# algbio/founderblockgraphs

Measured on AMD Instinct MI355X. Metric: MSA columns segmented/sec, higher is better.
Workload: dtype u32

## Files before the change

founderblockgraphs_amd/csrc/ctx.hip:

```cpp
#include "fbg_internal.h"
#include <chrono>
#include <stdarg.h>
#include <stdio.h>
#include <ctype.h>
#include <string.h>
#include <algorithm>
#include <atomic>
#include <thread>
#include <vector>

static std::string g_global_err;

int fbg_fail(fbg_ctx *ctx, int code, const char *fmt, ...)
{
    char buf[1024];
    va_list ap;
    va_start(ap, fmt);
    vsnprintf(buf, sizeof(buf), fmt, ap);
    va_end(ap);
    if (ctx) ctx->err = buf; else g_global_err = buf;
    return code;
}

int fbg_reserve(fbg_ctx *ctx, DevBuf &b, size_t bytes, std::vector<DevBuf *> *owner, bool accounted)
// ... 177 lines not shown
    {"span_slow_split", &FbgOptions::span_slow_split},
    {"poison", &FbgOptions::poison},
    {"dpw_matrix", &FbgOptions::dpw_matrix},
    {"dp_chain1", &FbgOptions::dp_chain1},
    {"msd_ext", &FbgOptions::msd_ext},
    {"rows_wave", &FbgOptions::rows_wave},
    {"pairs_in_scan", &FbgOptions::pairs_in_scan},
    {"runs_wave_min", &FbgOptions::runs_wave_min},
    {"wave_list_cap", &FbgOptions::wave_list_cap},
    {"cand_local_sort", &FbgOptions::cand_local_sort},
    {"cand_lds_cap", &FbgOptions::cand_lds_cap},
    {"cand_sort_check", &FbgOptions::cand_sort_check},
    {"tie_gallop", &FbgOptions::tie_gallop},
    {"cand_counts_fused", &FbgOptions::cand_counts_fused},
    {"tie_sample_loop", &FbgOptions::tie_sample_loop},
};

struct InfoKey { const char *name; int64_t (*get)(const fbg_ctx &); };
static const InfoKey g_info_keys[] = {
    {"grs_threshold", [](const fbg_ctx &c) -> int64_t { return c.grs_t; }},
    {"grs_redone", [](const fbg_ctx &c) -> int64_t { return (int64_t)c.grs_redone; }},
    {"dp_kind", [](const fbg_ctx &c) -> int64_t { return c.dp_kind; }},
    {"msd_decline", [](const fbg_ctx &c) -> int64_t { return c.diag.msd_decline; }},
    {"pass1_ahead", [](const fbg_ctx &c) -> int64_t { return c.diag.pass1_ahead; }},
    {"ext_pairs", [](const fbg_ctx &c) -> int64_t { return c.diag.ext_pairs; }},
    {"text_pairs", [](const fbg_ctx &c) -> int64_t { return c.diag.text_pairs; }},
    {"cand_inversions", [](const fbg_ctx &c) -> int64_t { return c.diag.cand_inversions; }},
    {"cand_local_sorted", [](const fbg_ctx &c) -> int64_t { return c.diag.cand_local_sorted; }},
    {"wave_runs", [](const fbg_ctx &c) -> int64_t { return c.diag.wave_runs; }},
    {"rank_lean_used", [](const fbg_ctx &c) -> int64_t { return c.diag.rank_lean_used; }},
    {"rank_lean_launched", [](const fbg_ctx &c) -> int64_t { return c.diag.rank_lean_launched; }},
    {"pairs_rb", [](const fbg_ctx &c) -> int64_t { return c.diag.pairs_rb; }},
    {"key_b", [](const fbg_ctx &c) -> int64_t { return c.key_b; }},
    {"key_K", [](const fbg_ctx &c) -> int64_t { return c.key_K; }},
    {"key_packed", [](const fbg_ctx &c) -> int64_t { return c.key_packed; }},
    {"key_compact", [](const fbg_ctx &c) -> int64_t { return c.key_compact; }},
    {"alloc_calls", [](const fbg_ctx &c) -> int64_t { return (int64_t)c.alloc_calls; }},
    {"alloc_us", [](const fbg_ctx &c) -> int64_t { return (int64_t)c.alloc_us; }},
    {"span_decline", [](const fbg_ctx &c) -> int64_t { return c.diag.sp_decline; }},
    {"span_key_flags_used", [](const fbg_ctx &c) -> int64_t { return c.ix.index_valid && c.ix.spanned() && c.ix.sp_key_flags_sorted; }},
    {"span_scan_used", [](const fbg_ctx &c) -> int64_t { return c.ix.index_valid && c.ix.spanned(); }},
// ... 118 lines not shown
        (void)hipStreamSynchronize(ctx->up_stream);
        for (auto &e : ctx->up_ev) if (e) (void)hipEventDestroy(e);
        (void)hipStreamDestroy(ctx->up_stream);
    }
    for (auto &t : ctx->timers) {
        if (t.start) (void)hipEventDestroy(t.start);
        if (t.stop) (void)hipEventDestroy(t.stop);
    }
    if (ctx->stager.base) {
        for (int i = 0; i < ctx->stager.nslots; i++) (void)hipEventDestroy(ctx->stager.ev[i]);
        delete[] ctx->stager.ev;
        (void)hipStreamDestroy(ctx->stager.stream);
        (void)hipHostFree(ctx->stager.base);
    }
    if (ctx->pin_pair) (void)hipHostFree(ctx->pin_pair);
    if (ctx->aux_fork) (void)hipEventDestroy(ctx->aux_fork);
    if (ctx->aux_join) (void)hipEventDestroy(ctx->aux_join);
    if (ctx->aux) (void)hipStreamDestroy(ctx->aux);
    if (ctx->own_stream) (void)hipStreamDestroy(ctx->stream);
    delete ctx;
}

const char *fbg_last_error(const fbg_ctx *ctx) { return ctx ? ctx->err.c_str() : g_global_err.c_str(); }

int fbg_set_stream(fbg_ctx *ctx, void *hip_stream)
{
    if (!ctx) return FBG_ERR_INVALID;
    FBG_HIP_TRY(ctx, hipStreamSynchronize(ctx->stream));
    if (ctx->own_stream) { (void)hipStreamDestroy(ctx->stream); ctx->own_stream = false; }
    if (hip_stream) {
// ... 376 lines not shown
```

founderblockgraphs_amd/csrc/fbg_internal.h:

```cpp
#pragma once
#include <cstring>
#include <cstdlib>
#include <hip/hip_runtime.h>
#include <stdint.h>
#include <string>
#include <vector>
#include "../../include/fbg_hip.h"

#define FBG_WAVE 64

struct DevBuf {
    void *p = nullptr;
    size_t cap = 0;
    bool listed = false;
    template <class T> T *as() const { return reinterpret_cast<T *>(p); }
};

struct Stager {
    void *base = nullptr;
    size_t slot_bytes = 0;
    int nslots = 0;
    hipEvent_t *ev = nullptr;
    hipStream_t stream = nullptr;
};

struct StageTimer {
    hipEvent_t start = nullptr, stop = nullptr;
    bool recorded = false;
    int launches = 0;
};

struct FbgOptions {
    int64_t no_ranked = 0, no_packed = 0, force_wide = 0, full_keys = 0, no_msd_sort = 0, msd_min = -1, bp_min = -1,
            record_scatter = 0, lcp_text = 0, no_aux_stream = 0, rank_no_threshold = 0, dp_literal = 0, dp_wave = 0,
            dp_safe_window = 0, dp_tile = 0, pure_scan = 0, gapped_rank = 0, part_tricks_off = 0, msd_sample_bins = 0, msd_min_force = 0, msd_probe = 0, msd_xcd = -1, rank_no_lean = 0, no_stream_upload = 0,
            span_scan = 0, span_key_flags = 0, span_slow_split = 0, poison = 0, dpw_matrix = 0, dp_chain1 = 0, msd_ext = 1, rows_wave = 0,
            pairs_in_scan = 1, runs_wave_min = 16, wave_list_cap = 0,
            cand_local_sort = 1, cand_lds_cap = 0, cand_sort_check = 0,
            tie_gallop = 1, cand_counts_fused = 1, tie_sample_loop = 1;
};

enum class IndexKind { none, record, ranked, gapped, span };

struct IndexState {
    bool index_valid = false;
    IndexKind kind = IndexKind::none;
    bool ranked() const { return kind == IndexKind::ranked; }
    bool granked() const { return kind == IndexKind::gapped || kind == IndexKind::span; }
    bool spanned() const { return kind == IndexKind::span; }
    uint32_t *sa_ptr = nullptr;
    uint64_t *rk_keys = nullptr;
    int rk_b = 0, rk_key_bits = 0, rk_K = 0;
    int rk_layout = 0, rk_pb = 0;
    bool grs_flagged = false;
// ... 2 lines not shown
    bool lcp_from_keys = false;
    bool grs_ties_done = false;
    uint32_t n_exc = 0;
    bool part_active = false;
    bool gpart = false;
    int part = 0, nparts = 1;
    uint64_t part_count = 0;
    uint64_t part_T = 0;
    uint32_t part_gmin = 0;
};

struct BuildDiag {
    int64_t msd_decline = -1;
    int pass1_ahead = 0;
    int64_t ext_pairs = -1, text_pairs = -1;
    int64_t wave_runs = -1;
    int64_t cand_inversions = -1;
    int cand_local_sorted = -1;
    int rank_lean_launched = 0;
    int rank_lean_used = 0;
    int pairs_rb = -1;
    int sp_decline = 0;
};

struct SortExtras {
    const uint64_t *ebits = nullptr;
    const uint32_t *payload = nullptr;
    bool key_flags = false;
};

struct MsdPlan;
struct fbg_ctx {
    int device = 0;
    FbgOptions opt;
    std::string err;
    hipStream_t stream = nullptr;
    bool own_stream = false;
    hipStream_t aux = nullptr;
    hipEvent_t aux_fork = nullptr, aux_join = nullptr;
    bool aux_pending = false;
    uint32_t *pin_pair = nullptr;
    Stager stager;
    StageTimer timers[FBG_STAGE_COUNT];

    const uint8_t *d_msa = nullptr;
    DevBuf msa_own;
    uint64_t m = 0, n = 0;
    int reversed = 0;
    bool gapfree = true;
    bool have_ignore = false;
    uint8_t ignore_tab[256] = {0};
    uint64_t N = 0;
    uint64_t byte_hist[256] = {0};
    bool allow_wide = false;
    uint32_t mp = 0;
    DevBuf text;
// ... 173 lines not shown
```

founderblockgraphs_amd/csrc/host/host_selftest.cpp:

```cpp
#include <cstdio>
#include <cstdlib>
#include <string>
#include <vector>
#include "fasta.hpp"
#include "xgfa.hpp"
#include "../tie_extent.h"

static int tie_extent_selftest()
{
    const uint32_t cap = 8192;
    std::vector<uint32_t> sizes;
    for (uint32_t s = 1; s <= 70; s++) sizes.push_back(s);
    for (uint32_t s = 8191; s <= 8194; s++) sizes.push_back(s);
    unsigned long long cases = 0;
    for (const uint32_t s : sizes)
        for (int where = 0; where < 3; where++) {
            const uint64_t before = where == 0 ? 0 : 37, after = where == 2 ? 0 : 29;
            std::vector<uint64_t> keys;
            for (uint64_t i = 0; i < before; i++) keys.push_back(10 + i / 3);
            const uint64_t key = 1000;
            for (uint32_t i = 0; i < s; i++) keys.push_back(key);
            for (uint64_t i = 0; i < after; i++) keys.push_back(2000 + i / 2);
            const uint64_t k0 = before;
            uint64_t reads = 0;
// ... 10 lines not shown
                reads = 0;
                const uint32_t got = fbg_tie_extent(k0, hi, cap, key, key_at);
                const uint64_t most = FBG_TIE_PROBE + 2 * 14;
                if (got != want || reads > most) {
                    std::printf("tie_extent differs: size %u position %d hi %llu: got %u, want %u, %llu reads\n", s, where,
                                (unsigned long long)hi, got, want, (unsigned long long)reads);
                    return 1;
                }
                cases++;
            }
        }
    std::printf("tie_extent ok %llu\n", cases);
    return 0;
}

int main(int argc, char **argv)
{
    if (argc == 2 && std::string(argv[1]) == "tie-extent") return tie_extent_selftest();
    if (argc < 6) {
        std::fprintf(stderr, "usage: %s FASTA GAP_LIMIT ELASTIC PATHS OUT.gfa [BOUNDARY ...]\n", argv[0]);
        return 2;
    }
    Msa msa;
    if (!read_msa(argv[1], std::atol(argv[2]), std::atoi(argv[3]) != 0, std::atoi(argv[4]) != 0, msa)) {
        std::fprintf(stderr, "cannot read %s\n", argv[1]);
        return 3;
    }
    std::printf("%llu %llu\n", (unsigned long long)msa.m, (unsigned long long)msa.n);
    if (argc == 6 || msa.m == 0) return 0;
    std::vector<uint64_t> boundaries;
    int first_boundary = 6;
    BlockGraph g;
// ... 28 lines not shown
```

founderblockgraphs_amd/csrc/suffix_sort.hip:

```cpp
#include "fbg_internal.h"
#include "text_cmp.h"
#include <rocprim/rocprim.hpp>
#include <utility>
#include <cmath>

#define SS_THREADS 256

using fbg_sort_config = rocprim::radix_sort_config<
    rocprim::default_config, rocprim::default_config,
    rocprim::radix_sort_onesweep_config<rocprim::kernel_config<512, 32>, rocprim::kernel_config<1024, 8>, 9,
                                        rocprim::block_radix_rank_algorithm::match>>;

#define PK_ITEMS 8
#define FBG_SEP 0x80
struct PackArgs {
    const uint8_t *T;
    uint64_t N;
    const uint8_t *code;
    int b, K, pb;
    uint64_t *keys;
    uint32_t *vals;
    uint64_t lo, hi, cap;
    int nohi;
    unsigned long long *counter;
// ... 108 lines not shown
    a.ebits = x.ebits; a.payload = x.payload;
    a.key_flags = x.key_flags ? ctx->sp_flagT.as<uint8_t>() : nullptr;
    const dim3 grid(fbg_blocks(a.N, SS_THREADS * PK_ITEMS)), block(SS_THREADS);
    hipStream_t st = ctx->stream;
#define FBG_PACK(C, L, F) hipLaunchKernelGGL((k_pack<C, L, F>), grid, block, 0, st, a)
    if (g.compact) {
        if (g.packed) { if (filter) FBG_PACK(true, FBG_SLOTS_PACKED, true); else FBG_PACK(true, FBG_SLOTS_PACKED, false); }
        else if (g.wide) { if (filter) FBG_PACK(true, FBG_SLOTS_WIDE, true); else FBG_PACK(true, FBG_SLOTS_WIDE, false); }
        else { if (filter) FBG_PACK(true, FBG_SLOTS_PAIRS, true); else FBG_PACK(true, FBG_SLOTS_PAIRS, false); }
    } else {
        if (filter) FBG_PACK(false, FBG_SLOTS_PAIRS, true); else FBG_PACK(false, FBG_SLOTS_PAIRS, false);
    }
#undef FBG_PACK
}

__global__ void k_sample_keys(const uint8_t *__restrict__ T, uint64_t N, const uint8_t *__restrict__ code, int b, int K,
                              int compact, uint64_t stride, uint64_t S, uint64_t *__restrict__ out)
{
    __shared__ uint8_t cd[256];
    if (threadIdx.x < 256) cd[threadIdx.x] = code[threadIdx.x];
    __syncthreads();
    const uint64_t i = (uint64_t)blockIdx.x * blockDim.x + threadIdx.x;
    if (i >= S) return;
    const uint64_t p = i * stride;
    uint64_t key = 0;
    bool dead = false;
    for (int k0 = 0; k0 < K; k0 += 8) {
        const uint64_t x = p + k0 < N ? fbg_load8(T, p + k0) : 0ull;
        for (int k = k0; k < K && k < k0 + 8; k++) {
            const uint32_t c = p + k < N ? cd[(x >> (8 * (k - k0))) & 255u] : (compact ? FBG_SEP : 0);
            dead = dead || (compact && (c & FBG_SEP));
            key = (key << b) | (dead ? 0u : c);
        }
    }
    out[i] = key;
}

__global__ void k_count_equal_neighbours(const uint64_t *__restrict__ keys, uint64_t S, unsigned long long *__restrict__ out)
{
    const uint64_t i = (uint64_t)blockIdx.x * blockDim.x + threadIdx.x;
    const bool eq = i + 1 < S && keys[i] == keys[i + 1];
    __shared__ uint32_t blk;
    if (threadIdx.x == 0) blk = 0;
    __syncthreads();
    const unsigned long long m = __ballot(eq);
    if ((threadIdx.x & 63) == 0 && m) atomicAdd(&blk, (uint32_t)__popcll(m));
    __syncthreads();
    if (threadIdx.x == 0 && blk) atomicAdd(out, (unsigned long long)blk);
}

// ... 508 lines not shown
        const unsigned hi = (unsigned)(g.pb + g.key_bits);
        if (hi == 64 && count < (1u << 23)) lo = 0;
        return with_tmp(ctx, [&](void *tmp, size_t &bytes) {
            return rocprim::radix_sort_keys<fbg_sort_config>(tmp, bytes, ka, kb, (size_t)count, lo, hi, st);
        });
    }
    uint32_t *va = ctx->valsA.as<uint32_t>(), *vb = ctx->valsB.as<uint32_t>() + out_offset;
    unsigned lo = g.wide ? (unsigned)g.pb : key_flags ? 2u : 0u;
    const unsigned hi = lo + (unsigned)g.key_bits;
    if (hi == 64 && count < (1u << 23)) lo = 0;
    return with_tmp(ctx, [&](void *tmp, size_t &bytes) {
        return rocprim::radix_sort_pairs<fbg_sort_config>(tmp, bytes, ka, kb, va, vb, (size_t)count, lo, hi, st);
    });
}

static int sample_says_similar(fbg_ctx *ctx, const KeyGeom &g, bool *similar, int *launches)
{
    const uint64_t N = ctx->N;
    hipStream_t st = ctx->stream;
    *similar = false;
    if (N < (1u << 22)) return FBG_OK;
    const uint64_t S = 1u << 20, stride = N / S;
    FBG_TRY(fbg_reserve(ctx, ctx->dp_g, S * 8));
    FBG_TRY(fbg_reserve(ctx, ctx->dp_h, S * 8));
    uint64_t *smp = ctx->dp_g.as<uint64_t>(), *srt = ctx->dp_h.as<uint64_t>();
    unsigned long long *d_count = ctx->scalars.as<unsigned long long>() + 8;
    FBG_HIP_TRY(ctx, hipMemsetAsync(d_count, 0, 8, st));
    hipLaunchKernelGGL(k_sample_keys, dim3(fbg_blocks(S, 256)), dim3(256), 0, st, ctx->text.as<uint8_t>(), N, g.d_code, g.b, g.K,
                       g.compact ? 1 : 0, stride, S, smp);
    FBG_TRY(with_tmp(ctx, [&](void *tmp, size_t &bytes) {
        return rocprim::radix_sort_keys(tmp, bytes, smp, srt, (size_t)S, 0u, (unsigned)g.key_bits, st);
    }));
    hipLaunchKernelGGL(k_count_equal_neighbours, dim3(fbg_blocks(S, 256)), dim3(256), 0, st, srt, S, d_count);
    unsigned long long twins = 0;
    FBG_HIP_TRY(ctx, hipMemcpyAsync(&twins, d_count, 8, hipMemcpyDeviceToHost, st));
    FBG_HIP_TRY(ctx, hipStreamSynchronize(st));
    *launches += 3;
    const double est = (double)twins * (double)N / ((double)S * (double)S);
    *similar = est > 0.5;
    return FBG_OK;
}

int fbg_suffix_sort(fbg_ctx *ctx)
{
    const uint64_t N = ctx->N;
    hipStream_t st = ctx->stream;
    FBG_TRY(fbg_stage_begin(ctx, FBG_STAGE_SUFFIX_SORT));
    int launches = 0;
    const uint8_t *T = ctx->text.as<uint8_t>();
    KeyGeom g;
    SortExtras x;

    if (ctx->gapfree && !ctx->have_ignore && !ctx->opt.no_ranked) {
        if (!fbg_msd_pre_geom(ctx, &g)) FBG_TRY(fbg_key_setup(ctx, true, &g, &launches));
    }
    if (ctx->gapfree && !ctx->have_ignore && !ctx->opt.no_ranked && g.compact) {
        bool similar = false;
        FBG_TRY(sample_says_similar(ctx, g, &similar, &launches));
        uint64_t *sorted = nullptr;
        int msd_ok = 0;
        FBG_TRY(fbg_msd_sort(ctx, g, &sorted, &msd_ok, &launches));
        if (!msd_ok) {
            FBG_TRY(fbg_reserve(ctx, ctx->keysA, N * 8));
            FBG_TRY(fbg_reserve(ctx, ctx->keysB, N * 8));
            if (!g.packed) {
                FBG_TRY(fbg_reserve(ctx, ctx->valsA, N * 4));
                FBG_TRY(fbg_reserve(ctx, ctx->valsB, N * 4));
            }
            PackArgs pa;
            pa.T = T; pa.N = N; pa.code = g.d_code; pa.b = g.b; pa.K = g.K; pa.pb = g.pb;
            pa.keys = ctx->keysA.as<uint64_t>(); pa.vals = ctx->valsA.as<uint32_t>();
            pa.lo = pa.hi = pa.cap = 0; pa.nohi = 1; pa.counter = nullptr;
            launch_pack(ctx, g, false, pa, x);
            launches++;
            FBG_TRY(sort_slots(ctx, g, false, N, 0));
            sorted = ctx->keysB.as<uint64_t>();
        }
        uint32_t *svals = g.packed ? nullptr : ctx->valsB.as<uint32_t>();
        int done = 0;
        if (!similar && ctx->opt.pure_scan != 1) FBG_TRY(fbg_rank_scan_try(ctx, sorted, svals, g, &done));
        if (!done && ctx->opt.pure_scan != -1) FBG_TRY(fbg_pure_scan_try(ctx, sorted, svals, g, &done));
        if (done) {
            FBG_HIP_TRY(ctx, hipGetLastError());
            return fbg_stage_end(ctx, FBG_STAGE_SUFFIX_SORT, launches);
        }
    }

    FBG_TRY(fbg_key_setup(ctx, false, &g, &launches));
    int b = g.b, K = g.K, key_bits = g.key_bits;
    FBG_TRY(fbg_reserve(ctx, ctx->keysA, N * 8));
    FBG_TRY(fbg_reserve(ctx, ctx->keysB, N * 8));
    FBG_TRY(fbg_reserve(ctx, ctx->valsA, N * 4));
    FBG_TRY(fbg_reserve(ctx, ctx->valsB, N * 4));
// ... 282 lines not shown
```

founderblockgraphs_amd/csrc/text_build.hip:

```cpp
#include "fbg_internal.h"

#define TB_THREADS 256
#define TB_ITEMS 8
#define TB_CHUNK (TB_THREADS * TB_ITEMS)

__device__ __forceinline__ uint32_t wave_incl_scan(uint32_t v)
{
    const int lane = threadIdx.x & 63;
#pragma unroll
    for (int d = 1; d < 64; d <<= 1) {
        uint32_t o = __shfl_up(v, d, 64);
        if (lane >= d) v += o;
    }
    return v;
}

__device__ __forceinline__ uint32_t block_excl_scan(uint32_t v, uint32_t *total, uint32_t *lds4)
{
    const int lane = threadIdx.x & 63, w = threadIdx.x >> 6;
    uint32_t inc = wave_incl_scan(v);
    if (lane == 63) lds4[w] = inc;
    __syncthreads();
    uint32_t base = 0, tot = 0;
#pragma unroll
// ... 141 lines not shown
    }
    if (lane == 0) { red[0][threadIdx.x >> 6] = nongap; red[1][threadIdx.x >> 6] = ign; }
    __syncthreads();
    if (sh[threadIdx.x]) atomicAdd(&hist[threadIdx.x], (unsigned long long)sh[threadIdx.x]);
    if (T_copy && threadIdx.x == 1 && x_hi == n) T_copy[i * (n + 1) + n] = '#';
    if (threadIdx.x == 0) {
        uint32_t a = 0, b = 0;
        for (int k = 0; k < TB_THREADS / 64; k++) { a += red[0][k]; b += red[1][k]; }
        atomicAdd(&tot[i], a);
        segcnt[i * gridDim.x + blockIdx.x] = a;
        atomicAdd(&scalars[0], (unsigned long long)((x_hi > x_lo ? x_hi - x_lo : 0) - a));
        if (b) atomicAdd(&scalars[1], (unsigned long long)b);
    }
}

__global__ void k_row_offsets(const uint32_t *__restrict__ tot, uint64_t m, uint32_t *__restrict__ pos,
                              unsigned long long *__restrict__ scalars)
{
    if (blockIdx.x != 0 || threadIdx.x >= 64) return;
    const uint64_t per = (m + 63) / 64, lo = min(m, (uint64_t)threadIdx.x * per), hi = min(m, lo + per);
    unsigned long long mine = 0;
    for (uint64_t i = lo; i < hi; i++) mine += (unsigned long long)tot[i] + 1;
    unsigned long long inc = mine;
    for (int d = 1; d < 64; d <<= 1) { const unsigned long long o = __shfl_up(inc, d, 64); if ((int)threadIdx.x >= d) inc += o; }
    unsigned long long s = inc - mine;
    for (uint64_t i = lo; i < hi; i++) { pos[i] = (uint32_t)s; s += (unsigned long long)tot[i] + 1; }
    if (threadIdx.x == 63) scalars[2] = inc + 1;
}

__global__ void k_seg_offsets(const uint32_t *__restrict__ segcnt, uint64_t m, uint32_t nseg, uint32_t *__restrict__ segoff)
// ... 162 lines not shown
#pragma unroll
        for (int k = 0; k < TB_ITEMS; k++)
            if (x0 + k < x_hi) igrow[i * n + x0 + k] = min(loc[k], right);
        __syncthreads();
        carry = chunk_min;
    }
}

int fbg_build_text(fbg_ctx *ctx, const uint8_t *ignore, uint64_t ignore_len)
{
    const uint64_t m = ctx->m, n = ctx->n;
    hipStream_t st = ctx->stream;
    FBG_TRY(fbg_stage_begin(ctx, FBG_STAGE_TEXT));
    int launches = 0;
    FBG_TRY(fbg_reserve(ctx, ctx->pos, m * 4));
    FBG_TRY(fbg_reserve(ctx, ctx->tot, m * 4));
    FBG_TRY(fbg_reserve(ctx, ctx->scalars, 256 * sizeof(unsigned long long)));
    FBG_TRY(fbg_reserve(ctx, ctx->small, 8192));
    FBG_HIP_TRY(ctx, hipMemsetAsync(ctx->scalars.p, 0, 64 * sizeof(unsigned long long), st));

    ctx->have_ignore = ignore_len > 0;
    ctx->cells_built = false;
    memset(ctx->ignore_tab, 0, sizeof(ctx->ignore_tab));
    if (ctx->have_ignore) {
        for (uint64_t k = 0; k < ignore_len; k++) ctx->ignore_tab[ignore[k]] = 1;
        FBG_HIP_TRY(ctx, hipMemcpyAsync(ctx->small.as<uint8_t>(), ctx->ignore_tab, 256, hipMemcpyHostToDevice, st));
    }
    unsigned long long *sc = ctx->scalars.as<unsigned long long>();
    unsigned long long *d_hist = reinterpret_cast<unsigned long long *>(ctx->small.as<uint8_t>() + 4096);
    FBG_HIP_TRY(ctx, hipMemsetAsync(d_hist, 0, 2048, st));
    FBG_HIP_TRY(ctx, hipMemsetAsync(ctx->tot.p, 0, m * 4, st));
    const unsigned nseg = (unsigned)((n + RC_SEG - 1) / RC_SEG);
    FBG_TRY(fbg_reserve(ctx, ctx->segtab, (size_t)m * nseg * 4 * 3));
    uint32_t *segcnt = ctx->segtab.as<uint32_t>(), *segoff = segcnt + (size_t)m * nseg;
    const bool fused = !ctx->reversed && n % 8 == 0 && ((uintptr_t)ctx->d_msa & 7) == 0 && m * (n + 1) + 1 < (1ull << 40);
    if (fused) FBG_TRY(fbg_reserve(ctx, ctx->text, m * (n + 1) + 1 + 64));
    const uint8_t *up = ctx->up_host;
    ctx->up_host = nullptr;
    ctx->pre_pass1 = false;
    if (up && fused && m >= 16) {
        constexpr int CHUNKS = 8;
        if (!ctx->up_stream) {
            FBG_HIP_TRY(ctx, hipStreamCreateWithFlags(&ctx->up_stream, hipStreamNonBlocking));
            for (auto &e : ctx->up_ev) FBG_HIP_TRY(ctx, hipEventCreateWithFlags(&e, hipEventDisableTiming));
        }
        uint8_t *d_msa = ctx->msa_own.as<uint8_t>();
        FBG_HIP_TRY(ctx, hipEventRecord(ctx->up_ev[CHUNKS], st));
        FBG_HIP_TRY(ctx, hipStreamWaitEvent(ctx->up_stream, ctx->up_ev[CHUNKS], 0));
        uint64_t r0s[CHUNKS + 1];
        for (int c = 0; c <= CHUNKS; c++) r0s[c] = m * c / CHUNKS;
        for (int c = 0; c < CHUNKS; c++) {
            FBG_HIP_TRY(ctx, hipMemcpyAsync(d_msa + r0s[c] * n, up + r0s[c] * n, (r0s[c + 1] - r0s[c]) * n, hipMemcpyHostToDevice, ctx->up_stream));
            FBG_HIP_TRY(ctx, hipEventRecord(ctx->up_ev[c], ctx->up_stream));
        }
        bool pre = false;
        for (int c = 0; c < CHUNKS; c++) {
            FBG_HIP_TRY(ctx, hipStreamWaitEvent(st, ctx->up_ev[c], 0));
            hipLaunchKernelGGL(k_row_count, dim3(nseg, (unsigned)(r0s[c + 1] - r0s[c])), dim3(TB_THREADS), 0, st, ctx->d_msa,
                               n, (const uint8_t *)nullptr, ctx->tot.as<uint32_t>(), sc, d_hist, segcnt, ctx->text.as<uint8_t>(), (uint32_t)r0s[c]);
            if (c == 0) {
                unsigned long long h0[1];
                FBG_HIP_TRY(ctx, hipMemcpyAsync(h0, sc, sizeof(h0), hipMemcpyDeviceToHost, st));
                FBG_HIP_TRY(ctx, hipMemcpyAsync(ctx->byte_hist, d_hist, 256 * sizeof(uint64_t), hipMemcpyDeviceToHost, st));
                FBG_HIP_TRY(ctx, hipStreamSynchronize(st));
                if (h0[0] == 0) {
                    for (int b = 0; b < 256; b++) ctx->byte_hist[b] = ctx->byte_hist[b] * m / r0s[1];
                    ctx->byte_hist['-'] = 0; ctx->byte_hist['#'] += m; ctx->byte_hist[0] += 1;
                    ctx->N = m * (n + 1) + 1;
                    ctx->gapfree = true;
                    FBG_HIP_TRY(ctx, hipMemsetAsync(ctx->text.as<uint8_t>() + ctx->N - 1, 0, 65, st));
                    int ok = 0;
                    FBG_TRY(fbg_msd_pre_begin(ctx, &ok));
                    pre = ok != 0;
                }
            }
            if (pre) FBG_TRY(fbg_msd_pre_pass1(ctx, c + 1 < CHUNKS ? r0s[c + 1] * (n + 1) : ctx->N));
        }
        ctx->pre_pass1 = pre;
        launches += CHUNKS - 1;
    } else {
        if (up) FBG_TRY(fbg_upload(ctx, ctx->msa_own.p, up, m * n));
        hipLaunchKernelGGL(k_row_count, dim3(nseg, (unsigned)m), dim3(TB_THREADS), 0, st, ctx->d_msa,
                           n, (const uint8_t *)nullptr, ctx->tot.as<uint32_t>(), sc, d_hist, segcnt, fused ? ctx->text.as<uint8_t>() : (uint8_t *)nullptr);
    }
    hipLaunchKernelGGL(k_row_offsets, dim3(1), dim3(64), 0, st, ctx->tot.as<uint32_t>(), m,
                       ctx->pos.as<uint32_t>(), sc);
    launches += 2;
    unsigned long long h[3];
    FBG_HIP_TRY(ctx, hipMemcpyAsync(h, sc, sizeof(h), hipMemcpyDeviceToHost, st));
    FBG_HIP_TRY(ctx, hipMemcpyAsync(ctx->byte_hist, d_hist, 256 * sizeof(uint64_t), hipMemcpyDeviceToHost, st));
    FBG_HIP_TRY(ctx, hipStreamSynchronize(st));
    ctx->byte_hist['-'] = 0;
    ctx->byte_hist['#'] += m;
    ctx->byte_hist[0] += 1;
    ctx->gapfree = h[0] == 0;
    ctx->N = h[2];
    if (ctx->pre_pass1) {
        bool same = ctx->gapfree && ctx->N == m * (n + 1) + 1 && ctx->byte_hist[0] == 1;
        for (int b = 0; b < 256 && same; b++) same = (ctx->byte_hist[b] != 0) == ((ctx->pre_symbols[b >> 6] >> (b & 63)) & 1ull);
        ctx->pre_pass1 = same;
    }
    if (ctx->N >= (1ull << 32) && !(ctx->allow_wide && ctx->gapfree && !ctx->reversed && !ctx->have_ignore && ctx->N < (1ull << 40)))
        return fbg_fail(ctx, FBG_ERR_TOO_LARGE, "text length %llu needs >32-bit positions (only the partitioned index of a "
                        "gap-free MSA, elastic scan, goes beyond)", h[2]);
    if (ctx->reversed && !ctx->gapfree)
        return fbg_fail(ctx, FBG_ERR_INVALID,
                        "the non-elastic scan needs gap-free rows (the reference drops rows with gaps when "
                        "--gap-limit=1, fbg.cpp:176-177); this MSA has %llu gap cells", h[0]);
    ctx->mp = (uint32_t)((m + 63) & ~63ull);

    const size_t tbytes = ctx->N + 64;
    FBG_TRY(fbg_reserve(ctx, ctx->text, tbytes));
    FBG_HIP_TRY(ctx, hipMemsetAsync(ctx->text.as<uint8_t>() + ctx->N - 1, 0, 65, st));
    uint8_t *T = ctx->text.as<uint8_t>();
    const uint32_t *pos = ctx->pos.as<uint32_t>(), *tot = ctx->tot.as<uint32_t>();
    if (!ctx->gapfree) {
        FBG_TRY(fbg_reserve(ctx, ctx->colT, ctx->N * 4));
        FBG_TRY(fbg_reserve(ctx, ctx->gwin_rows, ((ctx->N >> 7) + 2) * 2));
        hipLaunchKernelGGL(k_seg_offsets, dim3(fbg_blocks(m, 64)), dim3(64), 0, st, segcnt, m, nseg, segoff);
        hipLaunchKernelGGL((k_write_text<true, false>), dim3(nseg, (unsigned)m), dim3(TB_THREADS), 0, st, ctx->d_msa, n,
                           pos, tot, T, (uint32_t *)nullptr, ctx->colT.as<uint32_t>(), (const uint32_t *)segoff,
                           m < 65535 ? ctx->gwin_rows.as<uint16_t>() : (uint16_t *)nullptr);
        launches++;
    } else if (ctx->reversed) {
        hipLaunchKernelGGL((k_write_text<false, true>), dim3(1, (unsigned)m), dim3(TB_THREADS), 0, st, ctx->d_msa, n,
                           pos, tot, T, (uint32_t *)nullptr, (uint32_t *)nullptr, (const uint32_t *)nullptr, (uint16_t *)nullptr);
    } else if (!fused) {
        hipLaunchKernelGGL(k_copy_rows, dim3((unsigned)((n + CR_SEG - 1) / CR_SEG), (unsigned)m), dim3(TB_THREADS), 0, st,
// ... 72 lines not shown
```

Baseline: 65.27 million.

## Add fast row-count kernel, hash-based sample twin estimate, single front memset

```diff
diff --git a/founderblockgraphs_amd/csrc/ctx.hip b/founderblockgraphs_amd/csrc/ctx.hip
--- a/founderblockgraphs_amd/csrc/ctx.hip
+++ b/founderblockgraphs_amd/csrc/ctx.hip
@@ -215,6 +215,9 @@
     {"tie_gallop", &FbgOptions::tie_gallop},
     {"cand_counts_fused", &FbgOptions::cand_counts_fused},
     {"tie_sample_loop", &FbgOptions::tie_sample_loop},
+    {"row_count_fast", &FbgOptions::row_count_fast},
+    {"twin_hash", &FbgOptions::twin_hash},
+    {"front_one_fill", &FbgOptions::front_one_fill},
 };
 
 struct InfoKey { const char *name; int64_t (*get)(const fbg_ctx &); };
@@ -226,6 +229,7 @@
     {"pass1_ahead", [](const fbg_ctx &c) -> int64_t { return c.diag.pass1_ahead; }},
     {"ext_pairs", [](const fbg_ctx &c) -> int64_t { return c.diag.ext_pairs; }},
     {"text_pairs", [](const fbg_ctx &c) -> int64_t { return c.diag.text_pairs; }},
+    {"sample_twins", [](const fbg_ctx &c) -> int64_t { return c.diag.sample_twins; }},
     {"cand_inversions", [](const fbg_ctx &c) -> int64_t { return c.diag.cand_inversions; }},
     {"cand_local_sorted", [](const fbg_ctx &c) -> int64_t { return c.diag.cand_local_sorted; }},
     {"wave_runs", [](const fbg_ctx &c) -> int64_t { return c.diag.wave_runs; }},
@@ -374,6 +378,9 @@
         (void)hipHostFree(ctx->stager.base);
     }
     if (ctx->pin_pair) (void)hipHostFree(ctx->pin_pair);
+    if (ctx->pin_twins) (void)hipHostFree(ctx->pin_twins);
+    if (ctx->twin_ev) (void)hipEventDestroy(ctx->twin_ev);
+    if (ctx->pin_front) (void)hipHostFree(ctx->pin_front);
     if (ctx->aux_fork) (void)hipEventDestroy(ctx->aux_fork);
     if (ctx->aux_join) (void)hipEventDestroy(ctx->aux_join);
     if (ctx->aux) (void)hipStreamDestroy(ctx->aux);
diff --git a/founderblockgraphs_amd/csrc/fbg_internal.h b/founderblockgraphs_amd/csrc/fbg_internal.h
--- a/founderblockgraphs_amd/csrc/fbg_internal.h
+++ b/founderblockgraphs_amd/csrc/fbg_internal.h
@@ -37,7 +37,8 @@
             span_scan = 0, span_key_flags = 0, span_slow_split = 0, poison = 0, dpw_matrix = 0, dp_chain1 = 0, msd_ext = 1, rows_wave = 0,
             pairs_in_scan = 1, runs_wave_min = 16, wave_list_cap = 0,
             cand_local_sort = 1, cand_lds_cap = 0, cand_sort_check = 0,
-            tie_gallop = 1, cand_counts_fused = 1, tie_sample_loop = 1;
+            tie_gallop = 1, cand_counts_fused = 1, tie_sample_loop = 1,
+            row_count_fast = 1, twin_hash = 1, front_one_fill = 1;
 };
 
 enum class IndexKind { none, record, ranked, gapped, span };
@@ -70,6 +71,7 @@
     int64_t msd_decline = -1;
     int pass1_ahead = 0;
     int64_t ext_pairs = -1, text_pairs = -1;
+    int64_t sample_twins = -1;
     int64_t wave_runs = -1;
     int64_t cand_inversions = -1;
     int cand_local_sorted = -1;
@@ -96,6 +98,10 @@
     hipEvent_t aux_fork = nullptr, aux_join = nullptr;
     bool aux_pending = false;
     uint32_t *pin_pair = nullptr;
+    unsigned long long *pin_twins = nullptr;
+    hipEvent_t twin_ev = nullptr;
+    bool twin_pending = false;
+    unsigned long long *pin_front = nullptr;
     Stager stager;
     StageTimer timers[FBG_STAGE_COUNT];
 
diff --git a/founderblockgraphs_amd/csrc/host/host_selftest.cpp b/founderblockgraphs_amd/csrc/host/host_selftest.cpp
--- a/founderblockgraphs_amd/csrc/host/host_selftest.cpp
+++ b/founderblockgraphs_amd/csrc/host/host_selftest.cpp
@@ -5,6 +5,7 @@
 #include "fasta.hpp"
 #include "xgfa.hpp"
 #include "../tie_extent.h"
+#include "../twin_hash.h"
 
 static int tie_extent_selftest()
 {
@@ -48,8 +49,41 @@
     return 0;
 }
 
+static int twin_hash_selftest(const char *path, int bits, bool slots_only)
+{
+    FILE *fh = std::fopen(path, "rb");
+    if (!fh || bits < 1 || bits > 30) { std::fprintf(stderr, "twin-hash: cannot read %s, or BITS not in 1 .. 30\n", path); return 2; }
+    std::vector<uint64_t> keys;
+    uint64_t k;
+    while (std::fread(&k, 8, 1, fh) == 1) keys.push_back(k);
+    std::fclose(fh);
+    if (slots_only) {
+        for (const uint64_t key : keys) std::printf("%llu\n", (unsigned long long)fbg_twin_slot(key, bits));
+        return 0;
+    }
+    std::vector<uint64_t> table((1ull << bits) + 2, FBG_TWIN_EMPTY);
+    uint64_t *counters = table.data() + (1ull << bits);
+    uint64_t longest = 0;
+    for (const uint64_t key : keys) {
+        if (key == FBG_TWIN_EMPTY) { counters[1]++; continue; }
+        uint64_t probes = 0;
+        counters[0] += fbg_twin_insert(key, bits, [&](uint64_t slot, uint64_t kk) -> uint64_t {
+            if (slot >= (1ull << bits)) { std::fprintf(stderr, "twin-hash: slot %llu beyond the table\n", (unsigned long long)slot); std::exit(1); }
+            probes++;
+            const uint64_t seen = table[slot];
+            if (seen == FBG_TWIN_EMPTY) table[slot] = kk;
+            return seen;
+        });
+        if (probes > longest) longest = probes;
+    }
+    std::printf("twin_hash %llu %llu\n", (unsigned long long)fbg_twin_total(counters[0], counters[1]), (unsigned long long)longest);
+    return 0;
+}
+
 int main(int argc, char **argv)
 {
+    if (argc == 4 && (std::string(argv[1]) == "twin-hash" || std::string(argv[1]) == "twin-slots"))
+        return twin_hash_selftest(argv[2], std::atoi(argv[3]), std::string(argv[1]) == "twin-slots");
     if (argc == 2 && std::string(argv[1]) == "tie-extent") return tie_extent_selftest();
     if (argc < 6) {
         std::fprintf(stderr, "usage: %s FASTA GAP_LIMIT ELASTIC PATHS OUT.gfa [BOUNDARY ...]\n", argv[0]);
diff --git a/founderblockgraphs_amd/csrc/suffix_sort.hip b/founderblockgraphs_amd/csrc/suffix_sort.hip
--- a/founderblockgraphs_amd/csrc/suffix_sort.hip
+++ b/founderblockgraphs_amd/csrc/suffix_sort.hip
@@ -1,5 +1,6 @@
 #include "fbg_internal.h"
 #include "text_cmp.h"
+#include "twin_hash.h"
 #include <rocprim/rocprim.hpp>
 #include <utility>
 #include <cmath>
@@ -146,15 +147,8 @@
 #undef FBG_PACK
 }
 
-__global__ void k_sample_keys(const uint8_t *__restrict__ T, uint64_t N, const uint8_t *__restrict__ code, int b, int K,
-                              int compact, uint64_t stride, uint64_t S, uint64_t *__restrict__ out)
-{
-    __shared__ uint8_t cd[256];
-    if (threadIdx.x < 256) cd[threadIdx.x] = code[threadIdx.x];
-    __syncthreads();
-    const uint64_t i = (uint64_t)blockIdx.x * blockDim.x + threadIdx.x;
-    if (i >= S) return;
-    const uint64_t p = i * stride;
+__device__ __forceinline__ uint64_t sample_key(const uint8_t *__restrict__ T, uint64_t N, const uint8_t *cd, int b, int K, int compact, uint64_t p)
+{
     uint64_t key = 0;
     bool dead = false;
     for (int k0 = 0; k0 < K; k0 += 8) {
@@ -165,7 +159,41 @@
             key = (key << b) | (dead ? 0u : c);
         }
     }
-    out[i] = key;
+    return key;
+}
+
+__global__ void k_sample_keys(const uint8_t *__restrict__ T, uint64_t N, const uint8_t *__restrict__ code, int b, int K,
+                              int compact, uint64_t stride, uint64_t S, uint64_t *__restrict__ out)
+{
+    __shared__ uint8_t cd[256];
+    if (threadIdx.x < 256) cd[threadIdx.x] = code[threadIdx.x];
+    __syncthreads();
+    const uint64_t i = (uint64_t)blockIdx.x * blockDim.x + threadIdx.x;
+    if (i >= S) return;
+    out[i] = sample_key(T, N, cd, b, K, compact, i * stride);
+}
+
+__global__ __launch_bounds__(256) void k_sample_twins(const uint8_t *__restrict__ T, uint64_t N, const uint8_t *__restrict__ code, int b, int K,
+                                                      int compact, uint64_t stride, uint64_t S, unsigned long long *__restrict__ table, int bits)
+{
+    __shared__ uint8_t cd[256];
+    cd[threadIdx.x] = code[threadIdx.x];
+    __syncthreads();
+    const uint64_t i = (uint64_t)blockIdx.x * blockDim.x + threadIdx.x;
+    uint32_t twin = 0, ones = 0;
+    if (i < S) {
+        const uint64_t key = sample_key(T, N, cd, b, K, compact, i * stride);
+        if (key == FBG_TWIN_EMPTY) ones = 1;
+        else twin = fbg_twin_insert(key, bits, [&](uint64_t slot, uint64_t k) -> uint64_t {
+            return atomicCAS(&table[slot], (unsigned long long)FBG_TWIN_EMPTY, (unsigned long long)k);
+        });
+    }
+    unsigned long long *counters = table + (1ull << bits);
+    const unsigned long long mt = __ballot(twin), mo = __ballot(ones);
+    if ((threadIdx.x & 63) == 0) {
+        if (mt) atomicAdd(&counters[0], (unsigned long long)__popcll(mt));
+        if (mo) atomicAdd(&counters[1], (unsigned long long)__popcll(mo));
+    }
 }
 
 __global__ void k_count_equal_neighbours(const uint64_t *__restrict__ keys, uint64_t S, unsigned long long *__restrict__ out)
@@ -704,11 +732,57 @@
     });
 }
 
+static int sample_launch(fbg_ctx *ctx, const KeyGeom &g, int *launches)
+{
+    const uint64_t N = ctx->N;
+    hipStream_t st = ctx->stream;
+    ctx->twin_pending = false;
+    if (N < (1u << 22)) return FBG_OK;
+    constexpr int LOG_S = 20, BITS = LOG_S + FBG_TWIN_SPARE;
+    const uint64_t S = 1u << LOG_S, stride = N / S;
+    if (!ctx->pin_twins) {
+        FBG_HIP_TRY(ctx, hipHostMalloc(reinterpret_cast<void **>(&ctx->pin_twins), 2 * sizeof(unsigned long long), hipHostMallocDefault));
+        FBG_HIP_TRY(ctx, hipEventCreateWithFlags(&ctx->twin_ev, hipEventDisableTiming));
+    }
+    FBG_TRY(fbg_reserve(ctx, ctx->dp_g, ((1ull << BITS) + 2) * 8));
+    unsigned long long *table = ctx->dp_g.as<unsigned long long>();
+    FBG_HIP_TRY(ctx, hipMemsetAsync(table, 0xff, ((1ull << BITS) + 2) * 8, st));
+    hipLaunchKernelGGL(k_sample_twins, dim3(fbg_blocks(S, 256)), dim3(256), 0, st, ctx->text.as<uint8_t>(), N, g.d_code, g.b, g.K,
+                       g.compact ? 1 : 0, stride, S, table, BITS);
+    FBG_HIP_TRY(ctx, hipMemcpyAsync(ctx->pin_twins, table + (1ull << BITS), 2 * sizeof(unsigned long long), hipMemcpyDeviceToHost, st));
+    FBG_HIP_TRY(ctx, hipEventRecord(ctx->twin_ev, st));
+    ctx->twin_pending = true;
+    *launches += 1;
+    return FBG_OK;
+}
+
+static bool twins_say_similar(fbg_ctx *ctx, uint64_t twins)
+{
+    const uint64_t N = ctx->N, S = 1u << 20;
+    ctx->diag.sample_twins = (int64_t)twins;
+    const double est = (double)twins * (double)N / ((double)S * (double)S);
+    return est > 0.5;
+}
+
+static int sample_verdict(fbg_ctx *ctx, bool *similar)
+{
+    *similar = false;
+    if (!ctx->twin_pending) return FBG_OK;
+    ctx->twin_pending = false;
+    FBG_HIP_TRY(ctx, hipEventSynchronize(ctx->twin_ev));
+    *similar = twins_say_similar(ctx, fbg_twin_total(ctx->pin_twins[0], ctx->pin_twins[1]));
+    return FBG_OK;
+}
+
 static int sample_says_similar(fbg_ctx *ctx, const KeyGeom &g, bool *similar, int *launches)
 {
     const uint64_t N = ctx->N;
     hipStream_t st = ctx->stream;
     *similar = false;
+    if (ctx->opt.twin_hash) {
+        FBG_TRY(sample_launch(ctx, g, launches));
+        return sample_verdict(ctx, similar);
+    }
     if (N < (1u << 22)) return FBG_OK;
     const uint64_t S = 1u << 20, stride = N / S;
     FBG_TRY(fbg_reserve(ctx, ctx->dp_g, S * 8));
@@ -726,8 +800,7 @@
     FBG_HIP_TRY(ctx, hipMemcpyAsync(&twins, d_count, 8, hipMemcpyDeviceToHost, st));
     FBG_HIP_TRY(ctx, hipStreamSynchronize(st));
     *launches += 3;
-    const double est = (double)twins * (double)N / ((double)S * (double)S);
-    *similar = est > 0.5;
+    *similar = twins_say_similar(ctx, twins);
     return FBG_OK;
 }
 
@@ -746,7 +819,8 @@
     }
     if (ctx->gapfree && !ctx->have_ignore && !ctx->opt.no_ranked && g.compact) {
         bool similar = false;
-        FBG_TRY(sample_says_similar(ctx, g, &similar, &launches));
+        if (ctx->opt.twin_hash) FBG_TRY(sample_launch(ctx, g, &launches));
+        else FBG_TRY(sample_says_similar(ctx, g, &similar, &launches));
         uint64_t *sorted = nullptr;
         int msd_ok = 0;
         FBG_TRY(fbg_msd_sort(ctx, g, &sorted, &msd_ok, &launches));
@@ -767,6 +841,7 @@
             sorted = ctx->keysB.as<uint64_t>();
         }
         uint32_t *svals = g.packed ? nullptr : ctx->valsB.as<uint32_t>();
+        if (ctx->opt.twin_hash) FBG_TRY(sample_verdict(ctx, &similar));
         int done = 0;
         if (!similar && ctx->opt.pure_scan != 1) FBG_TRY(fbg_rank_scan_try(ctx, sorted, svals, g, &done));
         if (!done && ctx->opt.pure_scan != -1) FBG_TRY(fbg_pure_scan_try(ctx, sorted, svals, g, &done));
diff --git a/founderblockgraphs_amd/csrc/text_build.hip b/founderblockgraphs_amd/csrc/text_build.hip
--- a/founderblockgraphs_amd/csrc/text_build.hip
+++ b/founderblockgraphs_amd/csrc/text_build.hip
@@ -1,4 +1,5 @@
 #include "fbg_internal.h"
+#include <type_traits>
 
 #define TB_THREADS 256
 #define TB_ITEMS 8
@@ -179,6 +180,163 @@
     }
 }
 
+#define RCF_UNROLL 4
+__global__ __launch_bounds__(TB_THREADS) void k_row_count_fast(const uint8_t *__restrict__ msa, uint64_t n, uint32_t *__restrict__ tot,
+                                                               unsigned long long *__restrict__ scalars,
+                                                               unsigned long long *__restrict__ hist, uint32_t *__restrict__ segcnt,
+                                                               uint8_t *__restrict__ T_copy, uint32_t row0)
+{
+    typedef uint32_t u32x4 __attribute__((ext_vector_type(4)));
+    typedef u32x4 u32x4_a8 __attribute__((aligned(8)));
+    typedef u32x4 u32x4_a1 __attribute__((aligned(1)));
+    constexpr int RC_CAND = 6;
+    __shared__ uint32_t red[TB_THREADS / 64];
+    __shared__ uint32_t sh[256];
+    const uint64_t i = (uint64_t)blockIdx.y + row0;
+    const uint8_t *row = msa + i * n;
+    const uint64_t x_lo = (uint64_t)blockIdx.x * RC_SEG, x_hi = min(n, x_lo + RC_SEG);
+    const int lane = threadIdx.x & 63;
+    sh[threadIdx.x] = 0;
+    __syncthreads();
+    uint32_t nongap = 0;
+    auto count = [&](uint32_t c, bool valid) {
+        nongap += valid && c != '-';
+        unsigned long long rest = __ballot(valid);
+        while (rest) {
+            const int l = __ffsll((long long)rest) - 1;
+            const uint32_t v = __shfl(c, l, 64);
+            const unsigned long long same = __ballot(valid && c == v);
+            if (lane == l) atomicAdd(&sh[v], (uint32_t)__popcll(same));
+            rest &= ~same;
+        }
+    };
+    uint32_t cand[RC_CAND], pat[RC_CAND], pc[RC_CAND];
+    int nc = 1;
+    bool ascii = true;
+    {
+        const uint64_t x = x_lo + lane;
+        uint32_t c = x < x_hi ? (uint32_t)row[x] : 0x100u;
+        cand[0] = '-';
+        unsigned long long rest = __ballot(c < 0x100u && c != '-');
+#pragma unroll
+        for (int k = 1; k < RC_CAND; k++) {
+            cand[k] = 0x100u;
+            if (rest) {
+                const int l = __ffsll((long long)rest) - 1;
+                cand[k] = __shfl(c, l, 64);
+                rest &= ~__ballot(c == cand[k]);
+                nc = k + 1;
+                ascii = ascii && cand[k] < 0x80u;
+            }
+        }
+#pragma unroll
+        for (int k = 0; k < RC_CAND; k++) { pat[k] = 0x01010101u * (cand[k] & 0xffu); pc[k] = 0; }
+    }
+    const uint8_t *seg = row + x_lo;
+    uint8_t *tseg = T_copy + i * (n + 1) + x_lo;
+    const uint32_t nbytes = x_hi > x_lo ? (uint32_t)(x_hi - x_lo) : 0u, nunits = nbytes / 16;
+    uint32_t inv = 0;
+    auto body = [&](auto tag) {
+        constexpr int NC = decltype(tag)::value;
+        for (uint32_t q0 = 0; q0 < nunits; q0 += TB_THREADS * RCF_UNROLL) {
+            const uint32_t q = q0 + threadIdx.x;
+            u32x4 wv[RCF_UNROLL];
+#pragma unroll
+            for (int u = 0; u < RCF_UNROLL; u++) {
+                const uint32_t qq = q + (uint32_t)u * TB_THREADS;
+                wv[u] = (u32x4)(0x2d2d2d2du);
+                if (qq < nunits) wv[u] = *reinterpret_cast<const u32x4_a8 *>(seg + 16 * qq);
+            }
+#pragma unroll
+            for (int u = 0; u < RCF_UNROLL; u++) {
+                const uint32_t qq = q + (uint32_t)u * TB_THREADS;
+                if (qq < nunits) *reinterpret_cast<u32x4_a1 *>(tseg + 16 * qq) = wv[u];
+            }
+            uint32_t tm[NC], any = 0, sum = 0;
+#pragma unroll
+            for (int k = 0; k < NC; k++) tm[k] = 0;
+#pragma unroll
+            for (int u = 0; u < RCF_UNROLL; u++)
+#pragma unroll
+                for (int j = 0; j < 4; j++) {
+                    const uint32_t w = wv[u][j];
+                    any |= w;
+#pragma unroll
+                    for (int k = 0; k < NC; k++) tm[k] += (uint32_t)__popc(((w ^ pat[k]) + 0x7f7f7f7fu) & 0x80808080u);
+                }
+#pragma unroll
+            for (int k = 0; k < NC; k++) sum += tm[k];
+            const bool bad = !ascii || (any & 0x80808080u) != 0 || sum != (uint32_t)(NC - 1) * 16u * RCF_UNROLL;
+            if (!__ballot(bad)) {
+#pragma unroll
+                for (int k = 0; k < NC; k++) pc[k] += 16u * RCF_UNROLL - tm[k];
+#pragma unroll
+                for (int u = 0; u < RCF_UNROLL; u++) inv += q + (uint32_t)u * TB_THREADS < nunits ? 0u : 16u;
+            } else {
+#pragma clang loop unroll(disable)
+                for (int u = 0; u < RCF_UNROLL; u++) {
+                    const uint32_t qq = q + (uint32_t)u * TB_THREADS;
+                    const bool valid = qq < nunits;
+#pragma clang loop unroll(disable)
+                    for (int j = 0; j < 4; j++) {
+                        const uint32_t w = valid ? *reinterpret_cast<const uint32_t *>(seg + 16 * qq + 4 * j) : 0u;
+                        uint32_t hit = 0;
+#pragma unroll
+                        for (int k = 0; k < NC; k++) {
+                            const uint32_t d = w ^ pat[k];
+                            uint32_t z = ~(((d & 0x7f7f7f7fu) + 0x7f7f7f7fu) | d) & 0x80808080u;
+                            if (!valid) z = 0;
+                            pc[k] += (uint32_t)__popc(z);
+                            hit |= z;
+                        }
+                        const bool odd = valid && hit != 0x80808080u;
+                        if (__ballot(odd)) {
+#pragma clang loop unroll(disable)
+                            for (int bb = 0; bb < 4; bb++) count((w >> (8 * bb)) & 0xffu, odd && !((hit >> (8 * bb + 7)) & 1u));
+                        }
+                    }
+                }
+            }
+        }
+    };
+    switch (nc) {
+    case 1: body(std::integral_constant<int, 1>()); break;
+    case 2: body(std::integral_constant<int, 2>()); break;
+    case 3: body(std::integral_constant<int, 3>()); break;
+    case 4: body(std::integral_constant<int, 4>()); break;
+    case 5: body(std::integral_constant<int, 5>()); break;
+    default: body(std::integral_constant<int, 6>()); break;
+    }
+    pc[0] -= inv;
+#pragma unroll
+    for (int k = 0; k < RC_CAND; k++) {
+        if (k >= nc) break;
+        uint32_t v = pc[k];
+        for (int d = 32; d >= 1; d >>= 1) v += __shfl_down(v, d, 64);
+        if (lane == 0 && v) atomicAdd(&sh[cand[k]], v);
+        if (k > 0) nongap += lane == 0 ? v : 0u;
+    }
+    const uint64_t tail = x_lo + (uint64_t)nunits * 16 + threadIdx.x;
+    if (threadIdx.x < 64) {
+        const bool valid = tail < x_hi;
+        const uint32_t c = valid ? (uint32_t)row[tail] : 0u;
+        if (valid) T_copy[i * (n + 1) + tail] = (uint8_t)c;
+        count(c, valid);
+    }
+    for (int d = 32; d >= 1; d >>= 1) nongap += __shfl_down(nongap, d, 64);
+    if (lane == 0) red[threadIdx.x >> 6] = nongap;
+    __syncthreads();
+    if (sh[threadIdx.x]) atomicAdd(&hist[threadIdx.x], (unsigned long long)sh[threadIdx.x]);
+    if (threadIdx.x == 1 && x_hi == n) T_copy[i * (n + 1) + n] = '#';
+    if (threadIdx.x == 0) {
+        uint32_t a = 0;
+        for (int k = 0; k < TB_THREADS / 64; k++) a += red[k];
+        atomicAdd(&tot[i], a);
+        segcnt[i * gridDim.x + blockIdx.x] = a;
+        atomicAdd(&scalars[0], (unsigned long long)(nbytes - a));
+    }
+}
+
 __global__ void k_row_offsets(const uint32_t *__restrict__ tot, uint64_t m, uint32_t *__restrict__ pos,
                               unsigned long long *__restrict__ scalars)
 {
@@ -371,10 +529,16 @@
     FBG_TRY(fbg_stage_begin(ctx, FBG_STAGE_TEXT));
     int launches = 0;
     FBG_TRY(fbg_reserve(ctx, ctx->pos, m * 4));
-    FBG_TRY(fbg_reserve(ctx, ctx->tot, m * 4));
+    const bool one_fill = ctx->opt.front_one_fill != 0;
+    const size_t tot_bytes = (m * 4 + 7) & ~(size_t)7, hist_bytes = 256 * sizeof(unsigned long long), cnt_bytes = 8 * sizeof(unsigned long long);
+    FBG_TRY(fbg_reserve(ctx, ctx->tot, tot_bytes + hist_bytes + cnt_bytes));
     FBG_TRY(fbg_reserve(ctx, ctx->scalars, 256 * sizeof(unsigned long long)));
     FBG_TRY(fbg_reserve(ctx, ctx->small, 8192));
-    FBG_HIP_TRY(ctx, hipMemsetAsync(ctx->scalars.p, 0, 64 * sizeof(unsigned long long), st));
+    if (one_fill) {
+        if (!ctx->pin_front) FBG_HIP_TRY(ctx, hipHostMalloc(reinterpret_cast<void **>(&ctx->pin_front), hist_bytes + cnt_bytes, hipHostMallocDefault));
+        FBG_HIP_TRY(ctx, hipMemsetAsync(ctx->tot.p, 0, tot_bytes + hist_bytes + cnt_bytes, st));
+    } else
+        FBG_HIP_TRY(ctx, hipMemsetAsync(ctx->scalars.p, 0, 64 * sizeof(unsigned long long), st));
 
     ctx->have_ignore = ignore_len > 0;
     ctx->cells_built = false;
@@ -383,15 +547,28 @@
         for (uint64_t k = 0; k < ignore_len; k++) ctx->ignore_tab[ignore[k]] = 1;
         FBG_HIP_TRY(ctx, hipMemcpyAsync(ctx->small.as<uint8_t>(), ctx->ignore_tab, 256, hipMemcpyHostToDevice, st));
     }
-    unsigned long long *sc = ctx->scalars.as<unsigned long long>();
-    unsigned long long *d_hist = reinterpret_cast<unsigned long long *>(ctx->small.as<uint8_t>() + 4096);
-    FBG_HIP_TRY(ctx, hipMemsetAsync(d_hist, 0, 2048, st));
-    FBG_HIP_TRY(ctx, hipMemsetAsync(ctx->tot.p, 0, m * 4, st));
+    unsigned long long *d_hist = reinterpret_cast<unsigned long long *>(one_fill ? ctx->tot.as<uint8_t>() + tot_bytes : ctx->small.as<uint8_t>() + 4096);
+    unsigned long long *sc = one_fill ? d_hist + 256 : ctx->scalars.as<unsigned long long>();
+    if (!one_fill) {
+        FBG_HIP_TRY(ctx, hipMemsetAsync(d_hist, 0, 2048, st));
+        FBG_HIP_TRY(ctx, hipMemsetAsync(ctx->tot.p, 0, m * 4, st));
+    }
     const unsigned nseg = (unsigned)((n + RC_SEG - 1) / RC_SEG);
     FBG_TRY(fbg_reserve(ctx, ctx->segtab, (size_t)m * nseg * 4 * 3));
     uint32_t *segcnt = ctx->segtab.as<uint32_t>(), *segoff = segcnt + (size_t)m * nseg;
     const bool fused = !ctx->reversed && n % 8 == 0 && ((uintptr_t)ctx->d_msa & 7) == 0 && m * (n + 1) + 1 < (1ull << 40);
     if (fused) FBG_TRY(fbg_reserve(ctx, ctx->text, m * (n + 1) + 1 + 64));
+    const bool early_sentinel = one_fill && fused;
+    if (early_sentinel) FBG_HIP_TRY(ctx, hipMemsetAsync(ctx->text.as<uint8_t>() + m * (n + 1), 0, 65, st));
+    const bool fast = fused && ctx->opt.row_count_fast != 0;
+    auto launch_count = [&](unsigned rows, uint32_t r0) {
+        if (fast)
+            hipLaunchKernelGGL(k_row_count_fast, dim3(nseg, rows), dim3(TB_THREADS), 0, st, ctx->d_msa, n, ctx->tot.as<uint32_t>(), sc, d_hist,
+                               segcnt, ctx->text.as<uint8_t>(), r0);
+        else
+            hipLaunchKernelGGL(k_row_count, dim3(nseg, rows), dim3(TB_THREADS), 0, st, ctx->d_msa, n, (const uint8_t *)nullptr,
+                               ctx->tot.as<uint32_t>(), sc, d_hist, segcnt, fused ? ctx->text.as<uint8_t>() : (uint8_t *)nullptr, r0);
+    };
     const uint8_t *up = ctx->up_host;
     ctx->up_host = nullptr;
     ctx->pre_pass1 = false;
@@ -413,8 +590,7 @@
         bool pre = false;
         for (int c = 0; c < CHUNKS; c++) {
             FBG_HIP_TRY(ctx, hipStreamWaitEvent(st, ctx->up_ev[c], 0));
-            hipLaunchKernelGGL(k_row_count, dim3(nseg, (unsigned)(r0s[c + 1] - r0s[c])), dim3(TB_THREADS), 0, st, ctx->d_msa,
-                               n, (const uint8_t *)nullptr, ctx->tot.as<uint32_t>(), sc, d_hist, segcnt, ctx->text.as<uint8_t>(), (uint32_t)r0s[c]);
+            launch_count((unsigned)(r0s[c + 1] - r0s[c]), (uint32_t)r0s[c]);
             if (c == 0) {
                 unsigned long long h0[1];
                 FBG_HIP_TRY(ctx, hipMemcpyAsync(h0, sc, sizeof(h0), hipMemcpyDeviceToHost, st));
@@ -425,7 +601,7 @@
                     ctx->byte_hist['-'] = 0; ctx->byte_hist['#'] += m; ctx->byte_hist[0] += 1;
                     ctx->N = m * (n + 1) + 1;
                     ctx->gapfree = true;
-                    FBG_HIP_TRY(ctx, hipMemsetAsync(ctx->text.as<uint8_t>() + ctx->N - 1, 0, 65, st));
+                    if (!early_sentinel) FBG_HIP_TRY(ctx, hipMemsetAsync(ctx->text.as<uint8_t>() + ctx->N - 1, 0, 65, st));
                     int ok = 0;
                     FBG_TRY(fbg_msd_pre_begin(ctx, &ok));
                     pre = ok != 0;
@@ -437,16 +613,22 @@
         launches += CHUNKS - 1;
     } else {
         if (up) FBG_TRY(fbg_upload(ctx, ctx->msa_own.p, up, m * n));
-        hipLaunchKernelGGL(k_row_count, dim3(nseg, (unsigned)m), dim3(TB_THREADS), 0, st, ctx->d_msa,
-                           n, (const uint8_t *)nullptr, ctx->tot.as<uint32_t>(), sc, d_hist, segcnt, fused ? ctx->text.as<uint8_t>() : (uint8_t *)nullptr);
+        launch_count((unsigned)m, 0);
     }
     hipLaunchKernelGGL(k_row_offsets, dim3(1), dim3(64), 0, st, ctx->tot.as<uint32_t>(), m,
                        ctx->pos.as<uint32_t>(), sc);
     launches += 2;
     unsigned long long h[3];
-    FBG_HIP_TRY(ctx, hipMemcpyAsync(h, sc, sizeof(h), hipMemcpyDeviceToHost, st));
-    FBG_HIP_TRY(ctx, hipMemcpyAsync(ctx->byte_hist, d_hist, 256 * sizeof(uint64_t), hipMemcpyDeviceToHost, st));
-    FBG_HIP_TRY(ctx, hipStreamSynchronize(st));
+    if (one_fill) {
+        FBG_HIP_TRY(ctx, hipMemcpyAsync(ctx->pin_front, d_hist, hist_bytes + cnt_bytes, hipMemcpyDeviceToHost, st));
+        FBG_HIP_TRY(ctx, hipStreamSynchronize(st));
+        memcpy(ctx->byte_hist, ctx->pin_front, hist_bytes);
+        memcpy(h, ctx->pin_front + 256, sizeof(h));
+    } else {
+        FBG_HIP_TRY(ctx, hipMemcpyAsync(h, sc, sizeof(h), hipMemcpyDeviceToHost, st));
+        FBG_HIP_TRY(ctx, hipMemcpyAsync(ctx->byte_hist, d_hist, 256 * sizeof(uint64_t), hipMemcpyDeviceToHost, st));
+        FBG_HIP_TRY(ctx, hipStreamSynchronize(st));
+    }
     ctx->byte_hist['-'] = 0;
     ctx->byte_hist['#'] += m;
     ctx->byte_hist[0] += 1;
@@ -468,7 +650,8 @@
 
     const size_t tbytes = ctx->N + 64;
     FBG_TRY(fbg_reserve(ctx, ctx->text, tbytes));
-    FBG_HIP_TRY(ctx, hipMemsetAsync(ctx->text.as<uint8_t>() + ctx->N - 1, 0, 65, st));
+    if (!(early_sentinel && ctx->gapfree && ctx->N == m * (n + 1) + 1))
+        FBG_HIP_TRY(ctx, hipMemsetAsync(ctx->text.as<uint8_t>() + ctx->N - 1, 0, 65, st));
     uint8_t *T = ctx->text.as<uint8_t>();
     const uint32_t *pos = ctx->pos.as<uint32_t>(), *tot = ctx->tot.as<uint32_t>();
     if (!ctx->gapfree) {
diff --git a/founderblockgraphs_amd/csrc/twin_hash.h b/founderblockgraphs_amd/csrc/twin_hash.h
--- /dev/null
+++ b/founderblockgraphs_amd/csrc/twin_hash.h
@@ -0,0 +1,36 @@
+#pragma once
+#include <stdint.h>
+
+#if defined(__HIPCC__)
+#define FBG_TWIN_HD __host__ __device__
+#else
+#define FBG_TWIN_HD
+#endif
+
+#define FBG_TWIN_EMPTY 0xffffffffffffffffull
+#define FBG_TWIN_SPARE 1
+
+FBG_TWIN_HD inline uint64_t fbg_twin_slot(uint64_t key, int bits)
+{
+    return ((key ^ (key >> 29)) * 0x9E3779B97F4A7C15ull) >> (64 - bits);
+}
+
+FBG_TWIN_HD inline uint64_t fbg_twin_next(uint64_t slot, int bits) { return (slot + 1) & ((1ull << bits) - 1); }
+
+template <class Cas> FBG_TWIN_HD inline uint32_t fbg_twin_insert(uint64_t key, int bits, Cas cas)
+{
+    uint64_t slot = fbg_twin_slot(key, bits);
+    for (uint64_t probe = 0; probe < (1ull << bits); probe++) {
+        const uint64_t seen = cas(slot, key);
+        if (seen == FBG_TWIN_EMPTY) return 0;
+        if (seen == key) return 1;
+        slot = fbg_twin_next(slot, bits);
+    }
+    return 0;
+}
+
+FBG_TWIN_HD inline uint64_t fbg_twin_total(uint64_t counter0, uint64_t counter1)
+{
+    const uint64_t found = counter0 + 1, ones = counter1 + 1;
+    return found + (ones ? ones - 1 : 0);
+}
```

Result: faster. 67.32 million (median of 6 runs) (+3.1%).
